# rabbah/openwhisk

Hardware: AMD Instinct MI355X
Metric: scheduling decisions/sec (whole node) at 10k invokers, 1M-activation batch (higher is better)
Workload: dtype int32; 1 GPU; headline; invokers=10000, batches=18, batch=57748, releases=809625, cluster_size=1, slots=split, invoker_memory_mb=16384, slot_mb=16384, health=static, one exchange per step, health_disagreeing_ranks=0, health_exchange=local copy (one rank, no process group), parallelism=1 controller shard(s), 1 per GPU, 1 GPU(s)

## Files before the change

openwhisk_amd/balancer.py:

```python
from __future__ import annotations

import ctypes as C
from dataclasses import dataclass

import numpy as np

from . import _lib
from ._lib import (ERANGE, FLAG_OVERLOAD, HEALTHY, NONE, OFFLINE, THROW_INDEX, UNHEALTHY, UNRESPONSIVE, OwgsError,
                   owgs_config)

__all__ = ["GpuShardingContainerPoolBalancer", "InvokerHealth", "Action", "NONE", "THROW_INDEX", "FLAG_OVERLOAD",
           "HEALTHY", "UNHEALTHY", "UNRESPONSIVE", "OFFLINE", "OwgsError"]

MB = 1024 * 1024


@dataclass(frozen=True)
class InvokerHealth:

    id: int
    user_memory_bytes: int
    status: int = HEALTHY


# ... 801 lines not shown
                            status=None, status_stride=0, n_status=0, stream=None):
        vp = lambda x: C.c_void_p(int(x)) if x else None
        ao = np.ascontiguousarray(acq_off, dtype=np.int64)
        ro = np.ascontiguousarray(rel_off, dtype=np.int64)
        self._chk(self._L.owgs_replay_device_group(self._h, len(ao) - 1, _p(ao), _p(ro), vp(act), vp(rel_aid),
                                                   int(seq_base), vp(out_inv), vp(out_flags), vp(rel_flags),
                                                   vp(status), int(status_stride), int(n_status), vp(stream)))

    @staticmethod
    def replay_device_multi(shards, stream=None):
        from ._lib import owgs_replay_io

        k = len(shards)
        ios = (owgs_replay_io * k)()
        for j, (_, a) in enumerate(shards):
            ios[j] = owgs_replay_io(*[int(x) if x else 0 for x in a])
        hs = (C.c_void_p * k)(*[b._h for b, _ in shards])
        b0 = shards[0][0]
        b0._chk(b0._L.owgs_replay_device_multi(hs, k, ios, C.c_void_p(int(stream)) if stream else None))

    def snapshot(self):
        self._chk(self._L.owgs_snapshot(self._h))

    def restore(self, stream=None):
        self._chk(self._L.owgs_restore(self._h, C.c_void_p(int(stream)) if stream else None))

    def update_health_device(self, n: int, status_dev_ptr: int, stream=None):
        self._chk(self._L.owgs_update_health_device(self._h, n, C.c_void_p(int(status_dev_ptr)),
                                                    C.c_void_p(int(stream)) if stream else None))

    def selftest(self):
        self._chk(self._L.owgs_selftest(self._h))

    def stats(self) -> dict:
        out = (C.c_uint64 * 48)()
        self._chk(self._L.owgs_read_stats(self._h, out, 48))
        d = {"passes": out[0], "probes": out[1], "fallbacks": out[2], "long_walks": out[3], "chunks": out[4],
             "stops": out[5], "general_probes": out[6], "general_lanes": out[7], "redecided": out[31] & 0xFFFFFFFF}
        if out[31] >> 32:
            d["redecided_prewalk"] = out[31] >> 32
        if out[46] or out[47]:
            d["large_spec"], d["large_alone"] = out[46], out[47]
            d["large_cycles"] = {"releases": out[40], "speculation": out[41], "kept": out[42], "alone": out[43]}
        if any(out[28:31]) and not any(out[8:16]):
            d["redecide"] = {"cycles": out[28], "walk_rounds": out[29], "scans": out[30], "setup": out[20], "walk": out[21],
                             "apply": out[22], "scan": out[23]}
        if any(out[8:16]):
            names = ["batch", "chunk_start", "speculate", "tables_buckets", "validate", "commit", "worst_hot", "worst_lane"]
            d["cycles"] = {k: out[8 + i] for i, k in enumerate(names)}
            d["cycles"]["first_passes"] = d.pop("general_probes")
            d["cycles"]["later_passes"] = d.pop("general_lanes")
            walk = ["worst_long", "long_walks_worst_wave", "long_rounds", "conc_long", "conc_long_rounds",
                    "full_walks", "full_walk_rounds", "hot_rounds", "cyc_rounds_c1", "cyc_rounds_conc",
                    "worst_scan_push", "worst_barrier8", "worst_queue"]
            d["walks"] = {k: out[16 + i] for i, k in enumerate(walk[:10])}
            d["walks"].update({k: out[28 + i] for i, k in enumerate(walk[10:])})
            d["cycles"]["rel_sweep"] = out[26]
            d["cycles"]["ct_rebuild"] = out[27]
            d["kernel_cycles"] = {"state_load": out[40], "batches": out[41], "write_back": out[42]}
        return d
```

openwhisk_amd/csrc/owgs_host.cpp:

```cpp
#include "owgs_ctx.h"
#include "owgs_divq.h"

static int32_t d2i(double d) {
    if (d != d) return 0;
    if (d >= 2147483647.0) return 2147483647;
    if (d <= -2147483648.0) return (-2147483647 - 1);
    return (int32_t)d;
}

static int sync_status(owgs_ctx* c) {
    if (!c->status_stale) return OWGS_OK;
    HIPCHK(c, hipEventSynchronize(c->ev_status));
    if (!c->status.empty())
        HIPCHK(c, hipMemcpy(c->status.data(), c->d_status.p, c->status.size(), hipMemcpyDeviceToHost));
    c->status_stale = false;
    return OWGS_OK;
}

int order_on(owgs_ctx* c, hipStream_t s) {
    if (c->tail_valid && c->tail_stream != s) HIPCHK(c, hipStreamWaitEvent(s, c->ev_tail, 0));
    return OWGS_OK;
}
static int tail_mark(owgs_ctx* c, hipStream_t s) {
    if (!c->ev_tail) HIPCHK(c, c->ev_tail.create(hipEventDisableTiming));
// ... 297 lines not shown
    if (live > 0) {
        c->w_keys = std::move(nk);
        c->w_vals = std::move(nv);
        c->w_wkey = std::move(nw);
        c->w_cap = (int32_t)cap;
        c->w_live = live;
    }
    return OWGS_OK;
}

void base_args(owgs_ctx* c, OwgsEngineArgs& A) {
    memset(&A, 0, sizeof(A));
    A.permits = c->d_permits.p;
    A.n_slots = c->n_slots;
    A.pool_mode = c->pool_mode;
    A.usable = c->d_usable.p;
    A.n_ids = c->n_ids;
    A.pool_words = c->d_pool_words.p;
    A.nm = c->nm;
    A.nb = c->nb;
    A.hlist = c->d_hlist.p;
    A.hm = c->hm;
    A.hb = c->hb;
    A.shortcut_ok = c->shortcut_ok;
    A.ct_keys = c->d_ct_keys.p;
    A.ct_vals = c->d_ct_vals.p;
    A.ct_tmp = c->d_ct_tmp.p;
    A.ct_clast = c->d_clast.p;
    A.ovf = ovf_args(c);
    A.n_actions = (int32_t)c->a_mem.size();
    A.rng_seed = c->cfg.rng_seed;
    A.stats = c->d_stats.p;
    A.err = c->d_err.p;
    A.opts = (env_opts().opts & ~OWGS_OPT_WIDE_MEM) | (c->wide_mem ? OWGS_OPT_WIDE_MEM : 0);
    A.hwords = c->grp_hwords;
    A.hstride = c->grp_hstride;
    A.trace = nullptr;
    if (env_opts().trace) {
        const size_t n = (size_t)(OWGS_EW + 1) * 16384 * 2;
        if (c->d_trace.reserve(n) == hipSuccess && hipMemset(c->d_trace.p, 0, n * 8) == hipSuccess) A.trace = c->d_trace.p;
    }
}

#ifndef OWGS_WIDE_UNITS
#define OWGS_WIDE_UNITS 60000.0
#endif
static int32_t chunk_width(owgs_ctx* c) {
    if (c->cw_cache > 0) return c->cw_cache;
    double slot_mb = 0, act_mb = 0;
    const int32_t nm = std::min<int32_t>(c->nm, (int32_t)c->mem.size());
    for (int32_t i = 0; i < nm; ++i)
        slot_mb += (double)std::max<int64_t>(c->cfg.min_memory_bytes, c->mem[i] / std::max(c->cluster, 1)) / 1048576.0;
    int64_t live = 0;
    for (size_t a = 0; a < c->a_mem.size(); ++a)
        if (c->a_live[a]) {
            act_mb += c->a_mem[a];
            ++live;
        }
    const double units = live == 0 || act_mb <= 0 ? 1e9 : slot_mb / (act_mb / (double)live);
    int32_t cw = units >= OWGS_WIDE_UNITS ? OWGS_WL : std::min(units >= OWGS_WIDE_UNITS / 2 ? 256 : 192, OWGS_WL);
    const int v = env_opts().cw;
    if (v >= 64 && v <= OWGS_WL) cw = v;
    c->cw_cache = cw;
    return cw;
}

int run_prepass(owgs_ctx* c, OwgsEngineArgs& A, int32_t n_batches, const int64_t* acq_off, const int32_t* act,
// ... 2833 lines not shown
```

openwhisk_amd/csrc/owgs_internal.h:

```cpp
#pragma once
#include <stdint.h>

#ifndef OWGS_EW
#define OWGS_EW 7
#endif
#ifndef OWGS_LPW
#define OWGS_LPW 64
#endif
#define OWGS_ENT (OWGS_EW * 64)
#define OWGS_WL (OWGS_EW * OWGS_LPW)
#define OWGS_NT (OWGS_ENT + 64)
#ifndef OWGS_NBK_LOG2
#define OWGS_NBK_LOG2 10
#endif
#define OWGS_NBK (1 << OWGS_NBK_LOG2)
#ifndef OWGS_CTC
#define OWGS_CTC 4096
#endif
#define OWGS_LDS_BYTES (160 * 1024)

#define OWGS_AM_POS_MASK 0x7FFFu
#define OWGS_AM_POOL (1u << 30)
#define OWGS_AM_COK (1u << 31)
#define OWGS_AM_MEM_MASK 0x1FFFFu
// ... 7 lines not shown
#define OWGS_RMASK 0x3FFu
#define OWGS_REC_NONEXT OWGS_RMASK
#define OWGS_REC_NOHOT 0x3FF

#define OWGS_CT_SLOT_SHIFT 15
#define OWGS_CT_C_BITS 12
#define OWGS_CT_C_MASK 0xFFFu
#define OWGS_CT_TOMB 0xFFFFFFFFu
#define OWGS_MAX_SLOTS_CT 32767
#define OWGS_MAX_SLOTKEYS 131070
#define OWGS_MAX_CONC 4095
#define OWGS_MAX_OPS 524287
#define OWGS_MAX_MEM_MB 131071

#define OWGS_NONE_V (-1)
#define OWGS_THROW_V (-2)
#define OWGS_REL_NOSUCH_BIT 1
#define OWGS_REL_OVERFLOW_BIT 2
#define OWGS_REL_NOENTRY_BIT 4
#define OWGS_RR_NOINV 0x7FFFu

#define OWGS_PW_UNUSABLE (-1)
#define OWGS_PW_BADID (-2)

#define OWGS_ERR_CTAB_FULL 1
#define OWGS_ERR_BAD_STREAM 2
#define OWGS_ERR_OPS 4
#define OWGS_ERR_INTERNAL 8
#define OWGS_ERR_PERMITS 16
#define OWGS_ERR_GEOM 32
#define OWGS_ERR_RELRISK 64

#define OWGS_OPT_WIDE_MEM 2

#define OWGS_PLIM (1 << 29)
#define OWGS_PENC (1 << 30)

#define OWGS_ST_PASSES 0
#define OWGS_ST_PROBES 1
#define OWGS_ST_FALLBACKS 2
#define OWGS_ST_LONG 3
#define OWGS_ST_CHUNKS 4
#define OWGS_ST_STOPS 5
#define OWGS_NSTATS 48

#define OWGS_MULTI_MAX 8
#define OWGS_MULTI_DEV_MAX 64

#define OWGS_CT_LDS_FILL (OWGS_CTC - 256)
struct OwgsOvf {
    uint2* t;
    int32_t cap;
    int32_t* cnt;
    uint32_t* rc;
    int32_t* touched;
    int32_t* n_touched;
};

struct OwgsWatch {
    uint32_t* keys;
    uint32_t* vals;
    int32_t cap;
    int32_t* cnt;
    int32_t* wkey;
};
#define OWGS_W_Z 0x80000000u

struct OwgsEngineArgs {
    int32_t* permits;
    int32_t n_slots;
    int32_t pool_mode;
    const uint32_t* usable;
    int32_t n_ids;
    const int32_t* pool_words;
    int32_t nm, nb;
    const int32_t* hlist;
// ... 558 lines not shown
```

openwhisk_amd/csrc/owgs_kernels.hip:

```cpp
#include <hip/hip_runtime.h>
#include <hipcub/hipcub.hpp>

#include <atomic>

#include "owgs_device.h"
#include "owgs_divq.h"
#include "owgs_internal.h"
#include "owgs_launch.h"
#include "owgs_table.h"

#ifdef OWGS_VARIANT_NS
#define OWGS_SHARED 0
namespace OWGS_VARIANT_NS {
#else
#define OWGS_SHARED 1
#endif
#ifndef OWGS_GEOM
#define OWGS_GEOM(name) name
#endif

#define K_NONE 0
#define K_THROW 1
#define K_TARGET 2
#define K_FALLBACK 3
// ... 56 lines not shown
    int pt_on = 1;
#define PT(k)                                        \
    {                                                \
        const u64 _t = memtime_pinned();             \
        if (pt_on) pt_acc[k] += _t - pt_t;           \
        pt_t = _t;                                   \
    }
#else
#define PT_DECL
#define PT(k)
#endif

#define SC_LMIN 0
#define SC_IRR 2
#define SC_RRISK 3
#define SC_U0 4
#define SC_U1 5
#define SC_USED 6
#define SC_NLIVE 7
#define SC_NHOT 8
#define SC_CBWD 9
#define SC_OVF 13
#define SC_CLAST 12
#define SC_LQN 10
#define SC_LQH 11
#define SC_LFIN 14
#define SC_NEXT 15
#define SC_CFT (16 + 10 * OWGS_EW)
#ifndef CFT_LOG2
#define CFT_LOG2 6
#endif
#define CFT_N (1 << CFT_LOG2)
#define SC_N (SC_CFT + 2 * CFT_N)

#ifndef NHOT
#define NHOT 16
#endif
#define HOT_RANKS 64
#ifndef HOT_MIN
#define HOT_MIN 6
#endif
#define HOT_CONC 0x3E0
#ifndef HOT_CONC_ON
#define HOT_CONC_ON 0
#endif
static_assert(OWGS_WL < HOT_CONC, "pk1 and the concurrent hot marker share the 10-bit ext field");
#define OWGS_WROWS ((OWGS_WL + 63) / 64)
__host__ __device__ inline int wave_cap(int len, int w) {
    const int b = len / OWGS_EW, r = len % OWGS_EW;
    return min(OWGS_LPW, b + (w < r ? 1 : 0));
}
__host__ __device__ inline int wave_off(int len, int w) {
    const int b = len / OWGS_EW, r = len % OWGS_EW;
    return w * b + min(w, r);
}

__device__ __forceinline__ int ct_block(uint4 e01, uint4 e23, uint32_t key, uint32_t h, uint32_t* val, int* idx) {
    const bool h0 = e01.x == key, h1 = e01.z == key, h2 = e23.x == key, h3 = e23.z == key;
    const bool z = e01.x == 0u || e01.z == 0u || e23.x == 0u || e23.z == 0u;
    const bool hit = h0 || h1 || h2 || h3;
    const uint32_t v = h0 ? e01.y : h1 ? e01.w : h2 ? e23.y : e23.w;
    const int k = h0 ? 0 : h1 ? 1 : h2 ? 2 : 3;
    *val = hit ? v : 0u;
    *idx = hit ? (int)h + k : -1;
    return hit ? 1 : (z ? 0 : 2);
}
// ... 740 lines not shown
        if (threadIdx.x == 0) tail_early(OWGS_ERR_GEOM);
        if (A.stats_next && threadIdx.x < OWGS_NSTATS) A.stats_next[threadIdx.x] = 0ull;
        return;
    }
#ifdef OWGS_PROFILE
    const u64 tk0 = memtime_pinned();
#endif
    extern __shared__ uint4 lds_raw[];
    char* L = (char*)lds_raw;
    const OwgsLayout Y = owgs_layout(A.n_slots, pool_mode, A.n_ids, A.nm, A.nb);
    int32_t* P = (int32_t*)(L + LY_P);
    uint32_t* ub = (uint32_t*)(L + Y.pool);
    int16_t* pw = (int16_t*)(L + Y.pool);
    uint32_t* pc = (uint32_t*)(L + Y.pc);
    uint32_t* ccw = (uint32_t*)(L + LY_CCW);
    const uint32_t* stgC = (const uint32_t*)(L + LY_STGC);
    uint2* ct = (uint2*)(L + LY_CT);
    uint4* stgA = (uint4*)(L + LY_STGA);
    int32_t* stgX = (int32_t*)(L + LY_STGX);
    uint32_t* fst = (uint32_t*)(L + LY_FST);
    int32_t* spt = (int32_t*)(L + LY_SPT);
    uint32_t* bhead = (uint32_t*)(L + LY_BHEAD);
    int32_t* nextl = (int32_t*)(L + LY_NEXTL);
    int32_t* spc = (int32_t*)(L + LY_SPC);
    uint8_t* cdirty = (uint8_t*)(L + LY_CDIRTY);
    uint2* skey = (uint2*)(L + LY_SKEY);
    uint4* lq = (uint4*)(L + LY_LQ);
    uint4* fxa = (uint4*)(L + LY_FXA);
    uint4* hdir = (uint4*)(L + LY_HDIR);
    int32_t* hocc = (int32_t*)(L + LY_HDIR + 16u * NHOT);
    int32_t* hflag = (int32_t*)(L + LY_HDIR + 20u * NHOT);
    uint2* htab = (uint2*)(L + LY_HTAB);
    int32_t* hscr = (int32_t*)(L + LY_HSCR);
    const uint32_t* stgL = (const uint32_t*)(L + LY_STGL);
    uint32_t* rc = (uint32_t*)(L + LY_RC);
    int32_t* sc = (int32_t*)(L + LY_SC);
#ifdef OWGS_PROFILE
    int* spw = sc + 16;
    int* pfw = sc + 16 + 4 * OWGS_EW;
#endif

    const int tid = threadIdx.x, wave = IO ? OWGS_EW : tid >> 6, lane = tid & 63;
    constexpr bool io = IO;
    const int n_slots = A.n_slots, nm = A.nm, nb = A.nb;
    uint32_t mgm = owgs_divq_magic((uint32_t)max(nm, 1));
    uint32_t mgb = owgs_divq_magic((uint32_t)max(nb, 1));
    asm volatile("" : "+v"(mgm), "+v"(mgb));
    const DivPos dvm = div_pos(nm, mgm), dvb = div_pos(nb, mgb);
    const int words = (A.n_ids + 31) >> 5;

    uint32_t err = 0;
    constexpr int LB = 8;
    if (tid < SC_N)
        sc[tid] = (tid == SC_IRR || tid == SC_RRISK) ? 0
                                                     : ((tid < 4 || tid >= SC_CFT) ? OWGS_WL : (tid < 6 ? (int)0x80000000 : 0));
    const bool wide_mem = (A.opts & OWGS_OPT_WIDE_MEM) != 0;
    if (A.rel_bound || wide_mem) lds_sync();
    bool rrisk = false;
    constexpr int LB4 = 5;
    const int n4 = n_slots >> 2;
    auto slot_in = [&](int i, int v, uint32_t u, unsigned long long bnd) {
        if (v < -OWGS_PLIM || v >= OWGS_PLIM) err |= OWGS_ERR_PERMITS;
        const bool unusable = pool_mode == 0 && i < A.n_ids && !((u >> (i & 31)) & 1u);
        if (bnd) rrisk = rrisk || (long long)v + (long long)bnd >= (long long)OWGS_PLIM;
        return unusable ? v + OWGS_PENC : v;
    };
    for (int j0 = 0; j0 < n4; j0 += OWGS_NT * LB4) {
        int4 v[LB4];
        uint32_t u[LB4];
        ulonglong2 r0[LB4], r1[LB4];
#pragma unroll
        for (int k = 0; k < LB4; ++k) {
            const int j = j0 + k * OWGS_NT + tid;
            v[k] = j < n4 ? ((const int4*)A.permits)[j] : make_int4(0, 0, 0, 0);
            u[k] = (pool_mode == 0 && j < n4 && 4 * j < A.n_ids) ? A.usable[j >> 3] : ~0u;
            r0[k] = r1[k] = make_ulonglong2(0ull, 0ull);
            if (A.rel_bound && j < n4) {
                r0[k] = ((const ulonglong2*)A.rel_bound)[2 * j];
                r1[k] = ((const ulonglong2*)A.rel_bound)[2 * j + 1];
            }
        }
#pragma unroll
        for (int k = 0; k < LB4; ++k) {
            const int j = j0 + k * OWGS_NT + tid;
            if (j >= n4) continue;
            const int i = 4 * j;
            ((int4*)P)[j] = make_int4(slot_in(i, v[k].x, u[k], r0[k].x), slot_in(i + 1, v[k].y, u[k], r0[k].y),
                                      slot_in(i + 2, v[k].z, u[k], r1[k].x), slot_in(i + 3, v[k].w, u[k], r1[k].y));
// ... 41 lines not shown
                if (i >= OWGS_CTC) continue;
                ct[i] = make_uint2(kk[k], vv[k]);
                used += kk[k] != 0;
            }
        }
        if (used) atomicAdd(&sc[SC_USED], used);
        if (tid == 0 && A.ovf.cap > 0) sc[SC_OVF] = __hip_atomic_load(A.ovf.cnt, __ATOMIC_RELAXED, __HIP_MEMORY_SCOPE_AGENT);
    }
    for (int i = tid; i < (int)(LY_UNI_BYTES / 4); i += OWGS_NT) ((uint32_t*)(L + LY_UNI))[i] = 0u;
    lds_sync();
    if (tid == 0 && A.ct_clast) sc[SC_CLAST] = min(*A.ct_clast, sc[SC_USED]);
    if (pool_mode == 0 && wave == 0) {
        int carry = 0;
        for (int w0 = 0; w0 <= words; w0 += 64) {
            const int w = w0 + lane;
            const int c = w < words ? __popc(ub[w]) : 0;
            const int inc = wave_incl_scan(c);
            if (w <= words) pc[w] = (uint32_t)(carry + inc - c);
            carry += __builtin_amdgcn_readlane(inc, 63);
        }
    }
    EngineCtx E;
    E.P = P;
    E.ub = ub;
    E.pw = pw;
    E.pc = pc;
    E.pool_mode = pool_mode;
    E.n_ids = A.n_ids;
    E.nm = nm;
    E.nb = nb;

    uint32_t st_pass = 0, st_probe = 0, st_fb = 0, st_long = 0, st_chunk = 0, st_stop = 0, st_gprobe = 0, st_glane = 0;
    uint32_t st_ext = 0;
#ifdef OWGS_EXT_PROF
    u64 xp_cyc = 0, xp_rounds = 0, xp_scans = 0, xp_ph[4] = {0, 0, 0, 0};
#endif
#ifdef OWGS_TRACE
    int tr_n = 0;
#endif
    PT_DECL

    int io_b = 0;
    int64_t io_c0 = 0;
    const uint32_t stgA_lds = (uint32_t)(size_t)stgA, stgX_lds = (uint32_t)(size_t)stgX, stgL_lds = (uint32_t)(size_t)stgL,
                   stgC_lds = (uint32_t)(size_t)stgC;
    auto io_gather = [&](int sb, int cb) {
#pragma unroll
        for (int k = 0; k < OWGS_WROWS; ++k) {
            const uint32_t m0 = __builtin_amdgcn_readfirstlane(stgC_lds + (uint32_t)(cb * OWGS_WL + 64 * k) * 4u);
            if (64 * k + lane < OWGS_WL) {
                const uint32_t a = stgA[sb * OWGS_WL + 64 * k + lane].z & OWGS_REC_NOACT;
                const int ai = (int)a < A.n_actions ? (int)a : 0;
                lds_dma4_l2(&A.gcur[ai], m0);
            }
        }
    };
    auto io_locate = [&](int& bb, int64_t& c0) -> bool {
        while (bb < A.n_batches && c0 >= A.acq_off[bb + 1]) {
            ++bb;
            if (bb < A.n_batches) c0 = A.acq_off[bb];
        }
        return bb < A.n_batches;
    };
    auto io_dma = [&](int64_t c0, int buf, int gc) {
        const int64_t last = A.n_act - 1;
        const uint32_t* lx = A.lix + (int64_t)gc * OWGS_WL;
// ... 220 lines not shown
                if (rel_ovf) {
                    const int nt = __hip_atomic_load(A.ovf.n_touched, __ATOMIC_RELAXED, __HIP_MEMORY_SCOPE_AGENT);
                    for (int i2 = tid; i2 < nt; i2 += OWGS_ENT) {
                        const int oj = __hip_atomic_load(&A.ovf.touched[i2], __ATOMIC_RELAXED, __HIP_MEMORY_SCOPE_AGENT);
                        const uint32_t v = __hip_atomic_load(&A.ovf.rc[oj], __ATOMIC_RELAXED, __HIP_MEMORY_SCOPE_AGENT);
                        __hip_atomic_store(&A.ovf.rc[oj], 0u, __ATOMIC_RELAXED, __HIP_MEMORY_SCOPE_AGENT);
                        const int R = (int)(v & 0xFFFu);
                        const uint32_t cv = ovf_ld(A.ovf.t, oj).y;
                        const int c0 = (int)(cv & OWGS_CT_C_MASK), ops0 = ct_ops(cv);
                        const int j = min((int)(v >> 12), ops0);
                        const int ops1 = ops0 - j;
                        if (ops1 == 0) ovf_st(A.ovf.t, oj, OWGS_CT_TOMB, 0u);
                        else ovf_st_val(A.ovf.t, oj, ct_val((c0 + j) % R, ops1));
                    }
                    __builtin_amdgcn_fence(__ATOMIC_RELEASE, "workgroup");
                }
            }
            if (rel_ovf) {
                lds_sync();
                if (tid == 0) {
                    __hip_atomic_store(A.ovf.n_touched, 0, __ATOMIC_RELAXED, __HIP_MEMORY_SCOPE_AGENT);
                    __builtin_amdgcn_fence(__ATOMIC_RELEASE, "workgroup");
                }
            }
        }

        lds_sync();
#ifdef OWGS_PROFILE
        const u64 tb1 = memtime_pinned();
#endif
        if (kConc && ((sc[SC_USED] > OWGS_CTC / 2 && sc[SC_USED] >= sc[SC_CLAST] + OWGS_CTC / 8) ||
                      (A.ovf.cap > 0 && sc[SC_OVF] > A.ovf.cap / 2))) {
            const bool had_ovf = sc[SC_OVF] > 0;
            if (!io) {
                for (int ix = tid; ix < OWGS_CTC; ix += OWGS_ENT) {
                    const uint32_t k = ct[ix].x;
                    if (k != 0u && k != OWGS_CT_TOMB) {
                        const int j = atomicAdd(&sc[SC_NLIVE], 1);
                        A.ct_tmp[2 * j] = k;
                        A.ct_tmp[2 * j + 1] = ct[ix].y;
                    }
                }
                if (had_ovf)
                    for (int ix = tid; ix < A.ovf.cap; ix += OWGS_ENT) {
                        const uint2 e = ovf_ld(A.ovf.t, ix);
                        if (e.x != 0u) ovf_st(A.ovf.t, ix, 0u, 0u);
                        if (e.x != 0u && e.x != OWGS_CT_TOMB) {
                            const int j = atomicAdd(&sc[SC_NLIVE], 1);
                            A.ct_tmp[2 * j] = e.x;
                            A.ct_tmp[2 * j + 1] = e.y;
                        }
                    }
                asm volatile("s_waitcnt vmcnt(0)" ::: "memory");
            }
            lds_sync();
            const int nlive = sc[SC_NLIVE];
            for (int ix = tid; ix < OWGS_CTC; ix += OWGS_NT) {
                ct[ix] = make_uint2(0u, 0u);
            }
            lds_sync();
            const int nprim = min(nlive, 3 * OWGS_CTC / 4);
            if (!io) {
                for (int j = tid; j < nlive; j += OWGS_ENT) {
                    const uint32_t k = __hip_atomic_load(&A.ct_tmp[2 * j], __ATOMIC_RELAXED, __HIP_MEMORY_SCOPE_AGENT);
                    const uint32_t v = __hip_atomic_load(&A.ct_tmp[2 * j + 1], __ATOMIC_RELAXED, __HIP_MEMORY_SCOPE_AGENT);
                    if (j < nprim) {
                        int fresh = 0;
                        const int ix = ct_insertv(ct, k, &fresh);
                        ct[ix].y = v;
                    } else if (ovf_insert(A.ovf, k, v) < 0) {
                        err |= OWGS_ERR_CTAB_FULL;
                    }
                }
// ... 113 lines not shown
                    (a != (int)OWGS_REC_NOACT && cok && !stale && (gcw >> 15) == btag) ? (gcw & 0x7FFFu) : 0u;
                ccw[li] = st0;
            }

            const int hsx = maxc > 1 ? ext - HOT_CONC : ext;
            const int hs = (valid && hsx >= 0 && hsx < NHOT && !(A.opts & 1)) ? hsx : -1;
            if (hs >= 0) {
                if (occ == 0) {
                    hdir[hs] = make_uint4(__float_as_uint(dcm.rm), rc4.x, rc4.y, (uint32_t)slot | ((uint32_t)li << 17));
                    hflag[hs] = 0;
                    atomicMax(&sc[SC_NHOT], hs + 1);
                }
                if (nxt == (int)OWGS_REC_NONEXT) hocc[hs] = occ;
            }
            LDS_SYNC_T(1);
            const int nhot = sc[SC_NHOT];
            if (io) {
                io_gather((g + 1) % OWGS_NSTG, (g + 1) & 1);
                if (io_locate(io_b, io_c0)) {
                    io_dma(io_c0, (g + 2) % OWGS_NSTG, g + 2);
                    io_c0 += A.cw;
                }
            }

            int f = 0;
            PT(1);
            int kind = K_NONE, t = -1, ks = 0, cons = 0, s_t = 0, r = 0;
            uint32_t cw = 0, cval = 0;
            int cidx = -1;
            bool keep = false;
            while (f < len) {
                ++st_pass;
                const bool ovf_on = kConc && OWGS_OVF && sc[SC_OVF] > 0;
#ifdef OWGS_PROFILE
                const u64 tpass0 = memtime_pinned();
#ifdef OWGS_PROF_LATER
                pt_on = f > 0;
#endif
#endif
                const bool act = pending && li >= f;
                if (keep && maxc > 1 && cdirty[par * OWGS_WL + lead]) keep = false;
                const bool spec = act && !keep;
                const int resume = (spec && kind == K_TARGET && maxc == 1 && r == 0 && cok) ? s_t : 0;
                if (spec) {
                    kind = K_NONE;
                    t = -1;
                    ks = 0;
                    cons = 0;
                    s_t = 0;
                    r = 0;
                    cw = 0;
                    cval = 0;
                    cidx = -1;
                }
                int ws = 0, wpos = 0, wcum = 0;
#ifdef OWGS_PROFILE
                const u64 ts_beg = memtime_pinned();
                int pf_fast = 0, pf_gen = 0, pf_pre = 0;
#endif
                {
                    const int wr = (wave + OWGS_EW) % OWGS_EW;
                    for (int h = io ? 0 : wr + 1; h < nhot; h += OWGS_EW + 1) {
                        const uint4 d = hdir[h];
                        if (d.z & (OWGS_AM_THROW | OWGS_AM_EMPTY)) continue;
                        if (hflag[h] != f) continue;
                        const int hhome = (int)(d.y & OWGS_AM_POS_MASK), hstep = (int)((d.y >> 15) & OWGS_AM_POS_MASK);
// ... 671 lines not shown
                    const int hc = pool ? hb_e : hm_e;
#define OWGS_LAND(X)                                          \
    {                                                         \
        const int x_ = (X);                                   \
        if (x_ < 0 || x_ >= n_slots) {                        \
            kind = K_THROW;                                   \
        } else {                                              \
            t = x_;                                           \
            if (maxc > 1) {                                   \
                cidx = ct_find2(ct, A.ovf, ovf_on, ct_key(t, slot), &cval); \
            }                                                 \
        }                                                     \
    }
                    if (hc <= 0) {
                        kind = K_NONE;
                    } else if (seqp == nullptr && pool_mode == 0) {
                        const int k = (int)rng_index(A.rng_seed, A.seq_base + (u64)i, (uint32_t)hc);
                        OWGS_LAND(select_pool(E, pool ? A.n_ids - nb : 0, k, pool ? full_b : full_m));
                    } else {
                        const u64 seq = seqp ? seqp[i] : (A.seq_base + (u64)i);
                        const int k = (int)rng_index(A.rng_seed, seq, (uint32_t)hc);
                        OWGS_LAND(pool_mode == 0 ? select_usable(E, pool ? A.n_ids - nb : 0, k)
                                                   : A.hlist[(pool ? A.hm : 0) + k]);
                    }
#undef OWGS_LAND
                }
                const bool part = act && (kind == K_TARGET || kind == K_FALLBACK);
                if (spec && part) {
                    const int c0v = (int)(cval & OWGS_CT_C_MASK);
                    if (maxc == 1) cons = mem;
                    else if (kind == K_FALLBACK) cons = c0v >= 1 ? 0 : mem;
                    else cons = (ks < c0v) ? 0 : (small_mod(ks - c0v, maxc) == 0 ? mem : 0);
                }
                const int bk = part ? (int)(((uint32_t)t * 2654435761u) >> (32 - OWGS_NBK_LOG2)) : 0;
                static_assert(OWGS_NBK == (1 << OWGS_NBK_LOG2) && OWGS_WL <= 512, "power-of-two buckets; lane fields 10 bits");
                if (part) {
                    if (cons) atomicSub(&P[t], cons);
                    atomicMax(&fst[bk], (uint32_t)(OWGS_WL - li));
                    nextl[li] = (int)atomicExch(&bhead[bk], (uint32_t)(li + 1));
                    spc[li] = cons;
                    if (maxc > 1) skey[li] = make_uint2((uint32_t)slot, a != (int)OWGS_REC_NOACT ? (uint32_t)a : 0x80000000u | li);
                }
                const int cft = SC_CFT + par * CFT_N + (int)(((uint32_t)slot * 2654435761u) >> (32 - CFT_LOG2));
                if (act && maxc > 1 && kind == K_FALLBACK) atomicMin(&sc[cft], li);
                if (own && li < OWGS_WL) spt[li] = part ? t : -1;
                LDS_SYNC_T(3);
                PT(3);
                bool nf = false;
#ifdef OWGS_STOP_REASONS
                int why = 0;
#endif
                if (part) {
                    const bool first = fst[bk] == (uint32_t)(OWGS_WL - li);
                    bool fit = first || P[t] >= 0 || (maxc > 1 && kind == K_TARGET && cons == 0);
                    if (!fit && kind != K_FALLBACK) {
                        int pf = 0, tot = 0;
                        for (int j = (int)bhead[bk] - 1; j >= 0; j = nextl[j] - 1)
                            if (spt[j] == t) {
                                const int cj = spc[j];
                                tot += cj;
                                pf += j < li ? cj : 0;
                            }
                        fit = P[t] + tot - pf - cons >= 0;
                    }
                    bool kf;
                    if (maxc == 1) {
                        kf = fit || kind == K_FALLBACK;
                    } else {
                        const int cfb = sc[cft];
                        if (kind == K_FALLBACK) kf = first && cfb >= li;
                        else kf = fit && cfb > li;
                        if (kf && pk1 > f) {
                            for (int j = (int)bhead[bk] - 1; j >= 0; j = nextl[j] - 1)
                                if (j >= f && j < li && spt[j] == t) {
                                    const uint2 kj = skey[j];
                                    const uint32_t wid = a != (int)OWGS_REC_NOACT ? (uint32_t)a : 0x80000000u | li;
                                    if (kj.x == (uint32_t)slot && kj.y != wid) kf = false;
                                }
                        }
                    }
// ... 196 lines not shown
                        A.rel_rec[relx] = make_uint2(inv15 | ((uint32_t)mem << 15),
                                                     (uint32_t)slot | ((uint32_t)maxc << 17));
                    }
#endif
                    if (a != (int)OWGS_REC_NOACT && (nxt == (int)OWGS_REC_NONEXT || nxt >= l)) {
                        uint32_t ns = cw & 0x7FFFu;
                        if (cok) {
                            if (kind == K_TARGET) ns = (uint32_t)s_t;
                            else if (kind == K_FALLBACK) ns = maxc == 1 ? (uint32_t)n : fallback_cursor(t);
                        }
                        ccw[lead] = ((uint32_t)(occ + 1) << 15) | ns;
                        if (cok && a != (int)OWGS_REC_NOACT && ns != (cw & 0x7FFFu)) {
#ifndef OWGS_EXP_NOGCUR
                            A.gcur[a] = (btag << 15) | ns;
#endif
                            if (kind == K_FALLBACK && maxc > 1) {
                                sc[SC_CBWD] = g + 1;
                                asm volatile("s_waitcnt vmcnt(0)" ::: "memory");
                            }
                        }
                    }
                    if (maxc > 1 && (kind == K_TARGET || kind == K_FALLBACK)) {
                        const bool writer = kind == K_FALLBACK || nxt == (int)OWGS_REC_NONEXT || nxt >= l ||
                                            spt[nxt] != t;
                        if (writer) {
                            const int c0v = (int)(cval & OWGS_CT_C_MASK), ops0 = ct_ops(cval);
                            const int jn = kind == K_FALLBACK ? 1 : ks + 1;
                            const int c1 = jn <= c0v ? c0v - jn
                                                     : (maxc - 1 - small_mod(jn - c0v - 1, maxc));
                            const int ops1 = ops0 + jn;
                            if (ops1 > OWGS_MAX_OPS) err |= OWGS_ERR_OPS;
                            int ix = cidx;
                            const uint32_t key = ct_key(t, slot), nv = ct_val(c1, ops1);
                            if (ix < 0) {
                                uint32_t vv;
                                if (ovf_on) {
                                    const int oj = ovf_find(A.ovf, key, &vv);
                                    if (oj >= 0) ix = OWGS_CTC + oj;
                                }
                                if (ix < 0) {
                                    if (sc[SC_USED] < OWGS_CT_LDS_FILL || !OWGS_OVF || A.ovf.cap <= 0) {
                                        int fresh = 0;
                                        ix = ct_upsertv(ct, key, &fresh);
                                        if (fresh) atomicAdd(&sc[SC_USED], 1);
                                    } else {
                                        ix = ct_findv(ct, key, &vv);
                                    }
                                }
                                if (ix < 0 && OWGS_OVF && A.ovf.cap > 0) {
                                    const int oj = ovf_insert(A.ovf, key, nv);
                                    if (oj >= 0) {
                                        ix = OWGS_CTC + oj;
                                        atomicAdd(&sc[SC_OVF], 1);
                                    }
                                }
                            }
                            if (ix < 0) err |= OWGS_ERR_CTAB_FULL;
                            else if (ix < OWGS_CTC) ct[ix].y = nv;
                            else {
                                ovf_st_val(A.ovf.t, ix - OWGS_CTC, nv);
                                ovf_w = true;
                            }
                        }
                    }
                    if (kind == K_FALLBACK && maxc == 1 && r == 0) atomicMin(&sc[pool ? SC_U1 : SC_U0], mem - 1);
                    pending = false;
                }
#ifdef OWGS_PROF_COMMIT
                const u64 tc1 = memtime_pinned();
#endif
                if (part) {
                    if (li >= l && cons && !fixup) atomicAdd(&P[t], cons);
                    fst[bk] = 0u;
                    bhead[bk] = 0u;
                }
                if (act && li >= l) {
                    keep = !nf;
                    if (keep && fixup && part && kind != K_FALLBACK && sc[SC_NEXT] > 0) {
                        const uint32_t h1 = hsh((uint32_t)t), h2 = hsh((uint32_t)a);
                        const uint32_t* sw = (const uint32_t*)lq;
                        if (((sw[h1 >> 5] >> (h1 & 31u)) | (sw[64 + (h2 >> 5)] >> (h2 & 31u))) & 1u) keep = false;
                    }
                    if (!keep && hs >= 0) hflag[hs] = l;
                    if (!keep && maxc > 1) cdirty[(par ^ 1) * OWGS_WL + lead] = 1;
                }
                if (io && l >= len) asm volatile("s_waitcnt vmcnt(0)" ::: "memory");
#ifdef OWGS_PROF_COMMIT
                if (!io && lane == 0) {
                    const u64 tc2 = memtime_pinned();
                    atomicMax(&pfw[0], (int)(tc1 - tc0));
                    atomicMax(&pfw[1], (int)(tc2 - tc1));
                }
#endif
                if (tid < CFT_N) sc[SC_CFT + (par ^ 1) * CFT_N + tid] = OWGS_WL;
                if (tid == 0) {
                    sc[SC_LQN] = 0;
                    sc[SC_LQH] = 0;
                    sc[SC_NHOT] = 0;
                    sc[SC_LMIN + (par ^ 1)] = OWGS_WL;
                    if (l < len) ++st_stop;
                }
                if (!io && __ballot(ovf_w)) __builtin_amdgcn_fence(__ATOMIC_RELEASE, "workgroup");
                LDS_SYNC_T(5);
                PT(5);
#ifdef OWGS_PROFILE
#ifdef OWGS_PROF_COMMIT
                if (tid == 0) {
                    pt_x[0] += (u64)pfw[0];
                    pt_x[1] += (u64)pfw[1];
                    pfw[0] = 0;
                    pfw[1] = 0;
                }
#elif !defined(OWGS_PROF_SPLIT)
                if (tid == 0) pt_x[f == 0 ? 0 : 1] += memtime_pinned() - tpass0;
#endif
#endif
                f = l;
                par ^= 1;
            }
        }
        if (tid == 0) {
            sc[SC_U0] = (int)0x80000000;
            sc[SC_U1] = (int)0x80000000;
        }
        lds_sync();
    }

#ifdef OWGS_PROFILE
    const u64 tk2 = memtime_pinned();
#endif
    for (int i = tid; i < n_slots; i += OWGS_NT) {
        const int v = P[i];
        A.permits[i] = v >= OWGS_PLIM ? v - OWGS_PENC : v;
    }
    if (tid == 0 && A.ovf.cap > 0) __hip_atomic_store(A.ovf.cnt, sc[SC_OVF], __ATOMIC_RELAXED, __HIP_MEMORY_SCOPE_AGENT);
    if (tid == 0 && A.ct_clast) *A.ct_clast = sc[SC_CLAST];
    for (int i = tid; i < OWGS_CTC; i += OWGS_NT) {
        const uint2 e = ct[i];
        A.ct_keys[i] = e.x;
        A.ct_vals[i] = e.y;
    }
    if (A.out_copy_n16 > 0) {
        __syncthreads();
        __builtin_amdgcn_fence(__ATOMIC_ACQUIRE, "agent");
        for (int k = tid; k < A.out_copy_n16; k += OWGS_NT) A.out_copy_dst[k] = A.out_copy_src[k];
    }
    if (A.err_host || A.ovf_host) {
        if (tid == 0) sc[SC_IRR] = 0;
        lds_sync();
        if (err) atomicOr(&sc[SC_IRR], (int)err);
        lds_sync();
        if (tid == 0) {
            const int e = sc[SC_IRR];
            if (e) atomicOr(A.err, e);
            if (A.err_host) *A.err_host = __hip_atomic_load(A.err, __ATOMIC_RELAXED, __HIP_MEMORY_SCOPE_AGENT) | e;
            if (A.ovf_host) *A.ovf_host = sc[SC_OVF];
        }
        err = 0;
    }
    if (err) atomicOr(A.err, (int)err);
    if (A.stats_next && tid < OWGS_NSTATS) A.stats_next[tid] = 0ull;
#ifdef OWGS_PROFILE
    if (tid == 0 && A.stats) {
        asm volatile("s_waitcnt vmcnt(0)" ::: "memory");
        const u64 tk3 = memtime_pinned();
        atomicAdd(&A.stats[40], tk1 - tk0);
        atomicAdd(&A.stats[41], tk2 - tk1);
        atomicAdd(&A.stats[42], tk3 - tk2);
    }
#endif
    if (A.stats) {
        atomicAdd(&A.stats[OWGS_ST_PROBES], (u64)st_probe);
        if (lane == 0) atomicAdd(&A.stats[OWGS_ST_LONG], (u64)st_long);
        if (!io) {
            atomicAdd(&A.stats[OWGS_ST_FALLBACKS], (u64)st_fb);
#if !defined(OWGS_PROFILE) && !defined(OWGS_STOP_REASONS)
            atomicAdd(&A.stats[6], (u64)st_gprobe);
            atomicAdd(&A.stats[7], (u64)st_glane);
#endif
        }
#ifdef OWGS_PROFILE
        if (!io && lane == 0)
            for (int k = 2; k < 10; ++k) atomicAdd(&A.stats[16 + k], pw_c[k]);
        if (tid == 0) {
            atomicAdd(&A.stats[28], pw_c[10]);
            atomicAdd(&A.stats[29], pw_c[11]);
            atomicAdd(&A.stats[30], sc_prof_q);
            atomicAdd(&A.stats[26], pt_y[0]);
            atomicAdd(&A.stats[27], pt_y[1]);
            atomicAdd(&A.stats[16], pw_c[0]);
            atomicAdd(&A.stats[17], pt_x[2]);
            for (int k = 0; k < 8; ++k) atomicAdd(&A.stats[8 + k], pt_acc[k]);
            atomicAdd(&A.stats[6], pt_x[0]);
            atomicAdd(&A.stats[7], pt_x[1]);
        }
#endif
        if (io && lane == 0) atomicAdd(&A.stats[31], (u64)st_ext);
#ifdef OWGS_EXT_PROF
        if (io && lane == 0) {
            atomicAdd(&A.stats[28], xp_cyc);
            atomicAdd(&A.stats[29], xp_rounds);
            atomicAdd(&A.stats[30], xp_scans);
            for (int k = 0; k < 4; ++k) atomicAdd(&A.stats[20 + k], xp_ph[k]);
        }
#endif
        if (tid == 0) {
            atomicAdd(&A.stats[OWGS_ST_PASSES], (u64)st_pass);
            atomicAdd(&A.stats[OWGS_ST_CHUNKS], (u64)st_chunk);
            atomicAdd(&A.stats[OWGS_ST_STOPS], (u64)st_stop);
        }
    }
}

__device__ __forceinline__ bool owgs_io_wave() {
#ifdef OWGS_ROLE_ONLY
    return OWGS_ROLE_ONLY != 0;
#else
    return __builtin_amdgcn_readfirstlane((int)(threadIdx.x >> 6)) >= OWGS_EW;
#endif
}

struct OwgsEngineOne {
    OwgsEngineArgs a[1];
};
template <int FEAT>
__global__ __launch_bounds__(OWGS_NT, 1) void owgs_engine_kernel(OwgsEngineOne M) {
    if (owgs_io_wave()) owgs_engine_body<FEAT, true>(M.a[blockIdx.x]);
    else owgs_engine_body<FEAT, false>(M.a[blockIdx.x]);
}

// ... 533 lines not shown
```

Before: 40.00 million decisions/s.

## Pre-find concurrency-table entries on the I/O wave before commit

Worker lanes that will need a new concurrency-table entry queue their keys in LDS scratch during the speculate phase. The I/O wave then upserts up to 64 of them in one round, so the later commit step reads a precomputed index instead of running its own table lookup. The intent is to take serialized hash probing off the commit critical path. In exchange it adds an LDS queue, extra ballots and atomics, and placeholder entries with value zero that must be filtered during compaction and written out as tombstones; the feature is turned off when the watch table is active.

```diff
diff --git a/openwhisk_amd/balancer.py b/openwhisk_amd/balancer.py
--- a/openwhisk_amd/balancer.py
+++ b/openwhisk_amd/balancer.py
@@ -857,6 +857,11 @@
     def selftest(self):
         self._chk(self._L.owgs_selftest(self._h))
 
+    def entry_stats(self) -> dict:
+        out = (C.c_uint64 * 48)()
+        self._chk(self._L.owgs_read_stats(self._h, out, 48))
+        return {"prefound": out[32], "lane_found": out[33]}
+
     def stats(self) -> dict:
         out = (C.c_uint64 * 48)()
         self._chk(self._L.owgs_read_stats(self._h, out, 48))
diff --git a/openwhisk_amd/csrc/owgs_host.cpp b/openwhisk_amd/csrc/owgs_host.cpp
--- a/openwhisk_amd/csrc/owgs_host.cpp
+++ b/openwhisk_amd/csrc/owgs_host.cpp
@@ -353,7 +353,8 @@
     A.rng_seed = c->cfg.rng_seed;
     A.stats = c->d_stats.p;
     A.err = c->d_err.p;
-    A.opts = (env_opts().opts & ~OWGS_OPT_WIDE_MEM) | (c->wide_mem ? OWGS_OPT_WIDE_MEM : 0);
+    A.opts = (env_opts().opts & ~OWGS_OPT_WIDE_MEM) | (c->wide_mem ? OWGS_OPT_WIDE_MEM : 0) |
+             (c->w_cap > 0 ? OWGS_OPT_NO_PREFIND : 0);
     A.hwords = c->grp_hwords;
     A.hstride = c->grp_hstride;
     A.trace = nullptr;
diff --git a/openwhisk_amd/csrc/owgs_internal.h b/openwhisk_amd/csrc/owgs_internal.h
--- a/openwhisk_amd/csrc/owgs_internal.h
+++ b/openwhisk_amd/csrc/owgs_internal.h
@@ -63,6 +63,7 @@
 #define OWGS_ERR_RELRISK 64
 
 #define OWGS_OPT_WIDE_MEM 2
+#define OWGS_OPT_NO_PREFIND 4
 
 #define OWGS_PLIM (1 << 29)
 #define OWGS_PENC (1 << 30)
@@ -73,6 +74,8 @@
 #define OWGS_ST_LONG 3
 #define OWGS_ST_CHUNKS 4
 #define OWGS_ST_STOPS 5
+#define OWGS_ST_PREFOUND 32
+#define OWGS_ST_LANEFOUND 33
 #define OWGS_NSTATS 48
 
 #define OWGS_MULTI_MAX 8
diff --git a/openwhisk_amd/csrc/owgs_kernels.hip b/openwhisk_amd/csrc/owgs_kernels.hip
--- a/openwhisk_amd/csrc/owgs_kernels.hip
+++ b/openwhisk_amd/csrc/owgs_kernels.hip
@@ -112,6 +112,15 @@
 #endif
 #define CFT_N (1 << CFT_LOG2)
 #define SC_N (SC_CFT + 2 * CFT_N)
+#ifndef PF_CAP
+#define PF_CAP 64
+#endif
+#define PF_QCAP 256
+#define SC_PFN SC_N
+#define SC_PFOFF (SC_N + 1)
+static_assert(PF_CAP >= 1 && PF_CAP <= 64, "one round of the I/O wave, one key per lane");
+static_assert((((4u * SC_N) + 15u) & ~15u) >= 4u * (SC_N + 2), "SC_PFN and SC_PFOFF sit in the scalars' padding");
+static_assert(8u * PF_QCAP <= 4u * 64 * (OWGS_EW + 1), "the pre-find queue fits the hot-walk scratch");
 
 #ifndef NHOT
 #define NHOT 16
@@ -918,6 +927,7 @@
     int32_t* hflag = (int32_t*)(L + LY_HDIR + 20u * NHOT);
     uint2* htab = (uint2*)(L + LY_HTAB);
     int32_t* hscr = (int32_t*)(L + LY_HSCR);
+    uint2* pfq = (uint2*)(L + LY_HSCR);
     const uint32_t* stgL = (const uint32_t*)(L + LY_STGL);
     uint32_t* rc = (uint32_t*)(L + LY_RC);
     int32_t* sc = (int32_t*)(L + LY_SC);
@@ -940,6 +950,10 @@
     if (tid < SC_N)
         sc[tid] = (tid == SC_IRR || tid == SC_RRISK) ? 0
                                                      : ((tid < 4 || tid >= SC_CFT) ? OWGS_WL : (tid < 6 ? (int)0x80000000 : 0));
+    if (kConc && tid == 0) {
+        sc[SC_PFN] = 0;
+        sc[SC_PFOFF] = (A.opts & OWGS_OPT_NO_PREFIND) ? 1 : 0;
+    }
     const bool wide_mem = (A.opts & OWGS_OPT_WIDE_MEM) != 0;
     if (A.rel_bound || wide_mem) lds_sync();
     bool rrisk = false;
@@ -1047,6 +1061,7 @@
 
     uint32_t st_pass = 0, st_probe = 0, st_fb = 0, st_long = 0, st_chunk = 0, st_stop = 0, st_gprobe = 0, st_glane = 0;
     uint32_t st_ext = 0;
+    uint32_t st_pf = 0, st_pl = 0;
 #ifdef OWGS_EXT_PROF
     u64 xp_cyc = 0, xp_rounds = 0, xp_scans = 0, xp_ph[4] = {0, 0, 0, 0};
 #endif
@@ -1333,13 +1348,14 @@
         if (kConc && ((sc[SC_USED] > OWGS_CTC / 2 && sc[SC_USED] >= sc[SC_CLAST] + OWGS_CTC / 8) ||
                       (A.ovf.cap > 0 && sc[SC_OVF] > A.ovf.cap / 2))) {
             const bool had_ovf = sc[SC_OVF] > 0;
+            const bool pf_live = sc[SC_PFOFF] == 0;
             if (!io) {
                 for (int ix = tid; ix < OWGS_CTC; ix += OWGS_ENT) {
-                    const uint32_t k = ct[ix].x;
-                    if (k != 0u && k != OWGS_CT_TOMB) {
+                    const uint2 e = ct[ix];
+                    if (e.x != 0u && e.x != OWGS_CT_TOMB && !(pf_live && e.y == 0u)) {
                         const int j = atomicAdd(&sc[SC_NLIVE], 1);
-                        A.ct_tmp[2 * j] = k;
-                        A.ct_tmp[2 * j + 1] = ct[ix].y;
+                        A.ct_tmp[2 * j] = e.x;
+                        A.ct_tmp[2 * j + 1] = e.y;
                     }
                 }
                 if (had_ovf)
@@ -1519,6 +1535,7 @@
             while (f < len) {
                 ++st_pass;
                 const bool ovf_on = kConc && OWGS_OVF && sc[SC_OVF] > 0;
+                const bool pf_go = kConc && !ovf_on && sc[SC_PFOFF] == 0;
 #ifdef OWGS_PROFILE
                 const u64 tpass0 = memtime_pinned();
 #ifdef OWGS_PROF_LATER
@@ -2256,6 +2273,22 @@
                     else if (kind == K_FALLBACK) cons = c0v >= 1 ? 0 : mem;
                     else cons = (ks < c0v) ? 0 : (small_mod(ks - c0v, maxc) == 0 ? mem : 0);
                 }
+                if (kConc && !io) {
+                    if (cidx < -1) cidx = -1;
+                    const bool pf = pf_go && part && maxc > 1 && cidx < 0;
+                    const u64 pm = __ballot(pf);
+                    if (pm) {
+                        int qb = 0;
+                        if (lane == 0) qb = atomicAdd(&sc[SC_PFN], __popcll(pm));
+                        qb = __builtin_amdgcn_readfirstlane(qb);
+                        const int q = qb + (int)__builtin_amdgcn_mbcnt_hi((uint32_t)(pm >> 32),
+                                                                         __builtin_amdgcn_mbcnt_lo((uint32_t)pm, 0u));
+                        if (pf && q < PF_QCAP) {
+                            pfq[q] = make_uint2(ct_key(t, slot), 0xFFFFFFFFu);
+                            cidx = -2 - q;
+                        }
+                    }
+                }
                 const int bk = part ? (int)(((uint32_t)t * 2654435761u) >> (32 - OWGS_NBK_LOG2)) : 0;
                 static_assert(OWGS_NBK == (1 << OWGS_NBK_LOG2) && OWGS_WL <= 512, "power-of-two buckets; lane fields 10 bits");
                 if (part) {
@@ -2270,6 +2303,19 @@
                 if (own && li < OWGS_WL) spt[li] = part ? t : -1;
                 LDS_SYNC_T(3);
                 PT(3);
+                if (kConc && io) {
+                    const int npf = min(sc[SC_PFN], PF_CAP);
+                    if (npf > 0 && sc[SC_USED] + npf <= OWGS_CT_LDS_FILL) {
+                        int fresh = 0, ix = -1;
+                        if (lane < npf) {
+                            ix = ct_upsertv(ct, pfq[lane].x, &fresh);
+                            pfq[lane].y = (uint32_t)ix;
+                        }
+                        const u64 fm = __ballot(fresh != 0);
+                        if (fm && lane == 0) atomicAdd(&sc[SC_USED], __popcll(fm));
+                        st_pf += (uint32_t)__popcll(__ballot(ix >= 0));
+                    }
+                }
                 bool nf = false;
 #ifdef OWGS_STOP_REASONS
                 int why = 0;
@@ -2532,7 +2578,13 @@
                             if (ops1 > OWGS_MAX_OPS) err |= OWGS_ERR_OPS;
                             int ix = cidx;
                             const uint32_t key = ct_key(t, slot), nv = ct_val(c1, ops1);
+                            if (ix < -1) ix = (int)pfq[-2 - ix].y;
                             if (ix < 0) {
+#ifdef OWGS_PROF_ENTRY
+                                const u64 te0 = memtime_pinned();
+                                const u64 tem = __ballot(true);
+#endif
+                                ++st_pl;
                                 uint32_t vv;
                                 if (ovf_on) {
                                     const int oj = ovf_find(A.ovf, key, &vv);
@@ -2554,6 +2606,13 @@
                                         atomicAdd(&sc[SC_OVF], 1);
                                     }
                                 }
+#ifdef OWGS_PROF_ENTRY
+                                {
+                                    const u64 te1 = memtime_pinned();
+                                    if (lane == ffs64(tem))
+                                        atomicAdd(&A.stats[34 + max(wave, 4) - 4], (1ull << 40) | (te1 - te0));
+                                }
+#endif
                             }
                             if (ix < 0) err |= OWGS_ERR_CTAB_FULL;
                             else if (ix < OWGS_CTC) ct[ix].y = nv;
@@ -2596,6 +2655,7 @@
                 if (tid == 0) {
                     sc[SC_LQN] = 0;
                     sc[SC_LQH] = 0;
+                    if (kConc) sc[SC_PFN] = 0;
                     sc[SC_NHOT] = 0;
                     sc[SC_LMIN + (par ^ 1)] = OWGS_WL;
                     if (l < len) ++st_stop;
@@ -2635,9 +2695,10 @@
     }
     if (tid == 0 && A.ovf.cap > 0) __hip_atomic_store(A.ovf.cnt, sc[SC_OVF], __ATOMIC_RELAXED, __HIP_MEMORY_SCOPE_AGENT);
     if (tid == 0 && A.ct_clast) *A.ct_clast = sc[SC_CLAST];
+    const bool pf_live = kConc && sc[SC_PFOFF] == 0;
     for (int i = tid; i < OWGS_CTC; i += OWGS_NT) {
         const uint2 e = ct[i];
-        A.ct_keys[i] = e.x;
+        A.ct_keys[i] = (pf_live && e.x != 0u && e.y == 0u) ? OWGS_CT_TOMB : e.x;
         A.ct_vals[i] = e.y;
     }
     if (A.out_copy_n16 > 0) {
@@ -2696,6 +2757,10 @@
         }
 #endif
         if (io && lane == 0) atomicAdd(&A.stats[31], (u64)st_ext);
+        if (kConc) {
+            if (io && lane == 0) atomicAdd(&A.stats[OWGS_ST_PREFOUND], (u64)st_pf);
+            if (!io && st_pl) atomicAdd(&A.stats[OWGS_ST_LANEFOUND], (u64)st_pl);
+        }
 #ifdef OWGS_EXT_PROF
         if (io && lane == 0) {
             atomicAdd(&A.stats[28], xp_cyc);
```

Result: faster. 41.20 million decisions/s, median of 6 (+3.0%).
